# sql-machine-learning/elasticdl

Hardware: NVIDIA B200
Metric: deepfm_train_samples_per_sec (higher is better)
Workload: dtype f32

## Files before the change

elasticdl_b200/_lib.py:

```python
import ctypes
import os

from elasticdl_b200 import build as _build

MAX_SHARDS = 16
MAX_SEGS = 96

OK, EINVAL, ECUDA, ENOTFOUND, EWIDTH, ERANGE, ESTATE = 0, -1, -2, -3, -4, -5, -6


class Seg(ctypes.Structure):
    _fields_ = [
        ("table", ctypes.c_int32),
        ("n", ctypes.c_int32),
        ("ids_dev", ctypes.c_void_p),
        ("n_dev", ctypes.c_void_p),
        ("rows_dev", ctypes.c_void_p),
    ]


class DeepFMArgs(ctypes.Structure):
    _fields_ = [
        ("G", ctypes.c_int32), ("B", ctypes.c_int32),
        ("inv", ctypes.c_void_p), ("n_unique", ctypes.c_void_p),
        ("bet_wide", ctypes.c_void_p), ("bet_deep", ctypes.c_void_p),
        ("dense", ctypes.c_void_p), ("labels", ctypes.c_void_p),
        ("params", ctypes.c_void_p), ("grads", ctypes.c_void_p),
        ("gsum_wide", ctypes.c_void_p), ("gsum_deep", ctypes.c_void_p),
        ("loss", ctypes.c_void_p), ("logits", ctypes.c_void_p), ("scratch", ctypes.c_void_p),
    ]


class PSError(RuntimeError):
    def __init__(self, code, msg):
        super().__init__("b200ps error %d: %s" % (code, msg))
        self.code = code


class PSNotFound(PSError, KeyError):
    pass


class PSRangeError(PSError, ValueError):
    pass


_vp, _i, _i64, _f, _sz = ctypes.c_void_p, ctypes.c_int, ctypes.c_int64, ctypes.c_float, ctypes.c_size_t
_segp = ctypes.POINTER(Seg)
SYMBOLS = {
    "b200ps_last_error": (ctypes.c_char_p, []),
    "b200ps_abi_version": (_i, []),
    "b200ps_create": (_i, [_i, _i, ctypes.c_char_p, ctypes.c_char_p, _i, ctypes.c_uint, ctypes.POINTER(_vp)]),
    "b200ps_destroy": (_i, [_vp]),
    "b200ps_clone_view": (_i, [_vp, _i, ctypes.POINTER(_vp)]),
    "b200ps_shard_create_local": (_i, [_vp, _i, _i]),
    "b200ps_shard_export": (_i, [_vp, _i, _vp, _sz, ctypes.POINTER(_sz)]),
    "b200ps_shard_import": (_i, [_vp, _i, _vp, _sz]),
    "b200ps_table_register": (_i, [_vp, ctypes.c_char_p, _i, ctypes.c_char_p, _i64, ctypes.c_uint64]),
    "b200ps_table_register_pair": (_i, [_vp, ctypes.c_char_p, ctypes.c_char_p, ctypes.c_char_p, _i64, ctypes.c_uint64]),
    "b200ps_table_register_hashed": (_i, [_vp, ctypes.c_char_p, _i, ctypes.c_char_p, _i64, ctypes.c_uint64]),
    "b200ps_dense_register": (_i, [_vp, ctypes.c_char_p, _i, _i64, _i]),
    "b200ps_lookup": (_i, [_vp, ctypes.c_char_p]),
    "b200ps_commit": (_i, [_vp]),
    "b200ps_pull_rows": (_i, [_vp, _segp, _i, _vp]),
    "b200ps_set_rows": (_i, [_vp, _segp, _i, _vp]),
    "b200ps_pull_rows_pair": (_i, [_vp, _segp, ctypes.POINTER(_vp), _i, _vp]),
    "b200ps_push_rows_pair": (_i, [_vp, _segp, ctypes.POINTER(_vp), _i, _vp]),
    "b200ps_xchg_create": (_i, [_vp, _i, _i, ctypes.POINTER(ctypes.c_int32), ctypes.POINTER(ctypes.c_int32)]),
    "b200ps_xchg_pull": (_i, [_vp, _vp, _vp, _vp, _vp, _vp]),
    "b200ps_xchg_profile": (_i, [_vp, _vp, _vp, _vp, _vp, _vp, _vp, ctypes.POINTER(ctypes.c_float), _vp]),
    "b200ps_xchg_push": (_i, [_vp, _vp, _vp, _vp]),
    "b200ps_pull_dense": (_i, [_vp, _segp, _i, _vp]),
    "b200ps_set_dense": (_i, [_vp, _segp, _i, _vp]),
    "b200ps_slot_rows": (_i, [_vp, _i, _i, _segp, _i, _vp]),
    "b200ps_slot_dense": (_i, [_vp, _i, _i, _segp, _i, _vp]),
    "b200ps_push_begin": (_i, [_vp, _f, ctypes.POINTER(ctypes.c_int32), _vp]),
    "b200ps_push_rows": (_i, [_vp, _segp, _i, _vp]),
    "b200ps_push_dense": (_i, [_vp, _segp, _i, _vp]),
    "b200ps_push_dense_reduce": (_i, [_vp, _i, ctypes.POINTER(_vp), _i, _f, _vp]),
    "b200ps_push_end": (_i, [_vp, _vp, _vp]),
    "b200ps_bump_step": (_i, [_vp, _vp]),
    "b200ps_push_begin_shard": (_i, [_vp, _i, _f, ctypes.POINTER(ctypes.c_int32), _vp]),
    "b200ps_push_end_shard": (_i, [_vp, _i, _vp]),
    "b200ps_raw_register": (_i, [_vp, ctypes.c_char_p, _sz]),
    "b200ps_raw_ptr": (_i, [_vp, _i, _i, ctypes.POINTER(_vp), ctypes.POINTER(_sz)]),
    "b200ps_barrier": (_i, [_vp, _vp]),
    "b200ps_kernel_sgd": (_i, [_vp, _vp, _f, ctypes.c_longlong, _vp]),
    "b200ps_kernel_momentum": (_i, [_vp, _vp, _vp, _f, _i, _f, ctypes.c_longlong, _vp]),
    "b200ps_kernel_adam": (_i, [_vp, _vp, _vp, _vp, _f, ctypes.c_longlong, ctypes.c_longlong, _f, _f, _f, _vp, _vp]),
    "b200ps_kernel_adagrad": (_i, [_vp, _vp, _vp, _f, ctypes.c_longlong, _f, _vp]),
    "b200ps_unique_workspace": (_sz, [_i, _i64]),
    "b200ps_unique": (_i, [_vp, _vp, _i, _i64, _vp, _vp, _vp, _vp, _sz, _vp]),
    "b200ps_unique_bounded_workspace": (_sz, [_i, _i64, ctypes.POINTER(_i64)]),
    "b200ps_unique_bounded": (_i, [_vp, _vp, _i, _i64, ctypes.POINTER(_i64), _vp, _vp, _vp, _vp, _sz, _vp]),
    "b200ps_unique_bounded_i32": (_i, [_vp, _vp, _i, _i64, ctypes.POINTER(_i64), _vp, _vp, _vp, _vp, _sz, _vp]),
    "b200ps_unique_bounded_ex": (_i, [_vp, _vp, _i, _i, _i64, ctypes.POINTER(_i64), _vp, _vp, _vp, _vp, _sz, _i, _vp]),
    "b200ps_debug_buffer": (_i, [_vp, _sz]),
    "b200ps_unique_packed": (_i, [_vp, _vp, ctypes.POINTER(ctypes.c_int32), _i, _i64, ctypes.POINTER(_i64), _vp, _vp, _vp, _vp,
                                  _sz, _i, _vp]),
    "b200ps_packed_ids_bytes": (_sz, [ctypes.POINTER(ctypes.c_int32), _i, _i64]),
    "b200ps_segment_sum": (_i, [_vp, _vp, _vp, _i, _i64, _i, _vp, _vp]),
    "b200ps_gather_rows": (_i, [_vp, _vp, _vp, _i, _i64, _i, _vp, _vp]),
    "b200ps_shard_state": (_i, [_vp, _i, ctypes.POINTER(ctypes.c_int32), ctypes.POINTER(_i64), ctypes.POINTER(ctypes.c_int32)]),
    "b200ps_set_shard_state": (_i, [_vp, _i, ctypes.c_int32, _i64, ctypes.c_int32]),
    "b200ps_snapshot_state": (_i, [_vp, _vp, _vp]),
    "b200ps_try_init": (_i, [_vp, _i, ctypes.POINTER(_i)]),
    "b200ps_finish_init": (_i, [_vp, _i, ctypes.c_int32, _vp]),
    "b200ps_table_size": (_i, [_vp, _i, _i, ctypes.POINTER(_i64)]),
    "b200ps_table_ids": (_i, [_vp, _i, _i, _vp, _i64, ctypes.POINTER(_i64)]),
    "b200ps_check": (_i, [_vp]),
    "b200ps_launch_count": (_i64, [_vp]),
    "b200_deepfm_param_count": (_sz, [_i]),
    "b200_deepfm_fwd_bwd": (_i, [ctypes.POINTER(DeepFMArgs), _vp]),
    "b200_deepfm_forward": (_i, [ctypes.POINTER(DeepFMArgs), _vp]),
    "b200_deepfm_fwd_bwd_mma": (_i, [ctypes.POINTER(DeepFMArgs), _vp]),
    "b200_deepfm_mma_launch_count": (_i64, []),
    "b200_deepfm_launch_count": (_i64, []),
    "b200_deepfm_fwd_bwd_tile": (_i, [ctypes.POINTER(DeepFMArgs), _vp]),
    "b200_deepfm_forward_tile": (_i, [ctypes.POINTER(DeepFMArgs), _vp]),
    "b200_deepfm_publish_loss": (_i, [_vp, _vp, _i, _vp, _vp]),
    "b200_deepfm_tile_prologue": (_i, [ctypes.POINTER(DeepFMArgs), _vp]),
    "b200_deepfm_tile_main": (_i, [ctypes.POINTER(DeepFMArgs), _vp]),
    "b200_deepfm_tile_launch_count": (_i64, []),
    "b200_deepfm_tile_last_error": (ctypes.c_char_p, []),
    "b200feat_last_error": (ctypes.c_char_p, []),
    "b200feat_transform": (_i, [_vp, _i, _vp, _i, _vp, _i, _vp, _i, _i, _vp, _i, _i, _i64, _vp, _i, _vp, _vp]),
    "b200feat_hash_strings": (_i, [_vp, _i, _i64, _i64, _vp, _vp]),
    "b200feat_hash_ints": (_i, [_vp, _i64, _i64, _vp, _vp]),
    "b200feat_bucketize": (_i, [_vp, _i64, _vp, _i, _vp, _vp]),
    "b200feat_fingerprint64": (_i, [_vp, _i, _i64, _vp, _vp]),
    "b200feat_launch_count": (_i64, []),
}

_lib = None


def lib():
    global _lib
    if _lib is None:
        path = _build.LIB
        if not os.path.exists(path) or _build._stale():
            path = _build.build()
        handle = ctypes.CDLL(path)
        for name, (res, args) in SYMBOLS.items():
            fn = getattr(handle, name)
            fn.restype = res
            fn.argtypes = args
        if handle.b200ps_abi_version() != 1:
            raise ImportError("libb200ps.so ABI version mismatch")
        _lib = handle
    return _lib


def check(rc):
    if rc >= 0:
        return rc
    msg = lib().b200ps_last_error().decode("utf-8", "replace")
    if rc == ENOTFOUND:
        raise PSNotFound(rc, msg)
    if rc == ERANGE:
        raise PSRangeError(rc, msg)
    if rc in (EINVAL, EWIDTH):
        raise ValueError("b200ps error %d: %s" % (rc, msg))
    raise PSError(rc, msg)
```

elasticdl_b200/csrc/deepfm_tower2.cu:

```cuda
#include <cuda_runtime.h>

#include <cstdlib>
#include <string>

#include "../../include/b200_deepfm.h"

namespace {

constexpr int ND = B200_DEEPFM_NDENSE, D = B200_DEEPFM_DIM, H1 = B200_DEEPFM_H1, H2 = B200_DEEPFM_H2;
constexpr int WD_PAD = 16;
constexpr int TS = 32;
constexpr int THREADS = 256;
constexpr int NKP = 8;
constexpr int KPC = 40;
constexpr int NCOL = 320;
constexpr int XS = 324;
constexpr int RS = 39;
constexpr int RW = H1 + D + 2;
constexpr int MS = 44;
constexpr int MAXG = 38;

struct Layout {
  int in, o_wd, o_w1, o_b1, o_w2, o_b2, o_w3, total;
};
__host__ __device__ inline Layout layout(int G) {
  Layout l;
  l.in = ND + G * D;
  l.o_wd = 0;
  l.o_w1 = WD_PAD;
  l.o_b1 = l.o_w1 + H1 * l.in;
  l.o_w2 = l.o_b1 + H1;
  l.o_b2 = l.o_w2 + H2 * H1;
  l.o_w3 = l.o_b2 + H2;
  l.total = l.o_w3 + H2;
  return l;
}

long long g_launches = 0;
thread_local std::string g_msg;

constexpr int SM_W1X = NCOL * H1;
constexpr int SM_X = TS * XS;
constexpr int SM_P = NKP * RW * TS;
constexpr int SM_R = 2 * TS * RS;
constexpr int SM_WV = MAXG * TS;
constexpr int SM_SMALL = 128;
constexpr size_t SMEM_BYTES = (size_t)(SM_W1X + SM_X + SM_P + SM_R + SM_WV + SM_SMALL) * sizeof(float);

__device__ __forceinline__ void cp_async16(void* smem, const void* gmem) {
  const unsigned s = (unsigned)__cvta_generic_to_shared(smem);
  asm volatile("cp.async.cg.shared.global [%0], [%1], 16;" ::"r"(s), "l"(gmem) : "memory");
}
__device__ __forceinline__ void cp_async4(void* smem, const void* gmem) {
  const unsigned s = (unsigned)__cvta_generic_to_shared(smem);
  asm volatile("cp.async.ca.shared.global [%0], [%1], 4;" ::"r"(s), "l"(gmem) : "memory");
}
__device__ __forceinline__ void cp_async_wait_all() { asm volatile("cp.async.wait_all;" ::: "memory"); }

__host__ __device__ inline int w1x_src(const Layout& l, int G, int c, int j) {
  const int ndeep = G * D;
  if (c < ndeep) return l.o_w1 + j * l.in + ND + c;
  if (c >= MAXG * D && c < MAXG * D + ND) return l.o_w1 + j * l.in + (c - MAXG * D);
  if (c == MAXG * D + ND) return l.o_b1 + j;
  return -1;
}

__global__ void __launch_bounds__(256) k_tile_prep(b200_deepfm_args_t a, int n_params, float* w1x, int main_grid) {
  const long long stride = (long long)gridDim.x * blockDim.x;
  const long long tid = (long long)blockIdx.x * blockDim.x + threadIdx.x;
  if (tid == 0 && a.loss) *a.loss = 0.f;
  if (tid == 0 && blockIdx.y == 0) reinterpret_cast<int*>(w1x + NCOL * H1)[0] = main_grid;
  if (blockIdx.y == 0) {
    if (a.grads)
      for (long long i = tid; i < n_params; i += stride) a.grads[i] = 0.f;
    const Layout l = layout(a.G);
    for (long long i = tid; i < (long long)NCOL * H1; i += stride) {
      const int c = (int)(i / H1), j = (int)(i - (long long)c * H1);
      const int src = w1x_src(l, a.G, c, j);
      w1x[i] = src >= 0 ? a.params[src] : 0.f;
    }
  }
  if (a.gsum_deep == nullptr) return;
  for (int g = blockIdx.y; g < a.G; g += gridDim.y) {
    const int u = a.n_unique[g];
    float* gw = a.gsum_wide + (long long)g * a.B;
    float4* gd = reinterpret_cast<float4*>(a.gsum_deep + (long long)g * a.B * D);
    for (long long i = tid; i < u; i += stride) gw[i] = 0.f;
    for (long long i = tid; i < 2LL * u; i += stride) gd[i] = make_float4(0.f, 0.f, 0.f, 0.f);
  }
}

template <bool BACKWARD>
__global__ void __launch_bounds__(THREADS, 2) k_tower_tile(b200_deepfm_args_t a, const float* __restrict__ w1x_g) {
  extern __shared__ __align__(16) float smem[];
  float* W1x = smem;
  float* X = W1x + SM_W1X;
  float* P = X + SM_X;
  int* Rt0 = reinterpret_cast<int*>(P + SM_P);
  float* WV = reinterpret_cast<float*>(Rt0 + SM_R);
  float* small = WV + SM_WV;
  float* s_w2 = small;
  float* s_b2 = small + 64;
  float* s_w3 = small + 68;
  float* s_wd = small + 72;
  float* T = P;
  float* Mst = P + RW * TS + 64;

  const Layout l = layout(a.G);
  const int B = a.B, G = a.G;
  const int t = threadIdx.x, lane = t & 31, warp = t >> 5;
  {
    const float4* src = reinterpret_cast<const float4*>(w1x_g);
    float4* dst = reinterpret_cast<float4*>(W1x);
    for (int i = t; i < SM_W1X / 4; i += THREADS) dst[i] = src[i];
    for (int i = t; i < H2 * H1; i += THREADS) s_w2[i] = a.params[l.o_w2 + i];
    if (t < H2) { s_b2[t] = a.params[l.o_b2 + t]; s_w3[t] = a.params[l.o_w3 + t]; }
    if (t < ND) s_wd[t] = a.params[l.o_wd + t];
  }
  float2 acc0[H1 / 2], acc1[2];
  float sacc = 0.f;
#pragma unroll
  for (int j = 0; j < H1 / 2; ++j) acc0[j] = make_float2(0.f, 0.f);
  acc1[0] = acc1[1] = make_float2(0.f, 0.f);
  float loss_acc = 0.f;
  __syncthreads();

  const long long ntile = ((long long)B + TS - 1) / TS;
  auto fetch_ranks = [&](const long long tl, int* dst) {
    const long long bb0 = tl * TS;
    for (int i = t; i < G * TS; i += THREADS) {
      long long b = bb0 + (i & 31);
      if (b >= B) b = B - 1;
      cp_async4(dst + (i & 31) * RS + (i >> 5), a.inv + (long long)(i >> 5) * B + b);
    }
  };
  __shared__ int s_tile[2];
  int* tile_counter = reinterpret_cast<int*>(const_cast<float*>(w1x_g) + SM_W1X);
  if (t == 0) {
    s_tile[0] = (int)blockIdx.x;
    s_tile[1] = atomicAdd(tile_counter, 1);
  }
  int cur = 0;
  if ((long long)blockIdx.x < ntile) fetch_ranks(blockIdx.x, Rt0);
  cp_async_wait_all();
  __syncthreads();
  for (int iter = 0;; ++iter, cur ^= 1) {
    const int tile = s_tile[iter & 1], tile_next = s_tile[(iter + 1) & 1];
    if (tile >= ntile) break;
    const long long b0 = (long long)tile * TS;
    int* Rt = Rt0 + cur * (TS * RS);
    {
      const int npair = G * TS;
      constexpr int NFILL = (TS * 16 + THREADS - 1) / THREADS;
      float dv[NFILL];
#pragma unroll
      for (int jj = 0; jj < NFILL; ++jj) {
        const int i = t + THREADS * jj;
        const int s = i >> 4, c = i & 15;
        long long b = b0 + s;
        if (b >= B) b = B - 1;
        float v = c == ND ? 1.0f : 0.f;
        if (i < TS * 16 && c < ND) v = a.dense[b * ND + c];
        dv[jj] = v;
      }
      const int nchunk = G * 2;
      for (int i = t; i < TS * nchunk; i += THREADS) {
        const int s = i / nchunk, ch = i - s * nchunk;
        const int g = ch >> 1;
        const int r = Rt[s * RS + g];
        cp_async16(X + s * XS + ch * 4, a.bet_deep + ((long long)g * B + r) * D + (ch & 1) * 4);
      }
      for (int i = t; i < npair; i += THREADS) {
        const int g = i >> 5, s = i & 31;
        cp_async4(WV + g * TS + s, a.bet_wide + (long long)g * B + Rt[s * RS + g]);
      }
      if (tile_next < ntile) fetch_ranks(tile_next, Rt0 + (cur ^ 1) * (TS * RS));
#pragma unroll
      for (int jj = 0; jj < NFILL; ++jj) {
        const int i = t + THREADS * jj;
        if (i < TS * 16) X[(i >> 4) * XS + MAXG * D + (i & 15)] = dv[jj];
      }
      for (int i = t; i < TS * (MAXG - G) * D; i += THREADS) {
        const int s = i / ((MAXG - G) * D), c = G * D + i % ((MAXG - G) * D);
        X[s * XS + c] = 0.f;
      }
      cp_async_wait_all();
    }
    __syncthreads();
    if (t == 0) s_tile[iter & 1] = atomicAdd(tile_counter, 1);
    const bool live = b0 + lane < B;
    {
      float2 h2[H1 / 2];
#pragma unroll
      for (int j = 0; j < H1 / 2; ++j) h2[j] = make_float2(0.f, 0.f);
      float sd[D], q = 0.f, lin = 0.f;
#pragma unroll
      for (int d = 0; d < D; ++d) sd[d] = 0.f;
      const float* xrow = X + lane * XS;
      const int c0 = warp * KPC;
#pragma unroll
      for (int gi = 0; gi < KPC / D; ++gi) {
        const int c = c0 + gi * D;
        const float4 xa = *reinterpret_cast<const float4*>(xrow + c);
        const float4 xb = *reinterpret_cast<const float4*>(xrow + c + 4);
        const float xv[D] = {xa.x, xa.y, xa.z, xa.w, xb.x, xb.y, xb.z, xb.w};
        const int g = c / D;
        if (g < G) {
#pragma unroll
          for (int d = 0; d < D; ++d) { sd[d] += xv[d]; q = fmaf(xv[d], xv[d], q); }
          lin += WV[g * TS + lane];
        } else if (c == MAXG * D) {
#pragma unroll
          for (int d = 0; d < D; ++d) lin = fmaf(s_wd[d], xv[d], lin);
        } else if (c == MAXG * D + D) {
#pragma unroll
          for (int d = 0; d < ND - D; ++d) lin = fmaf(s_wd[D + d], xv[d], lin);
        }
#pragma unroll
        for (int d = 0; d < D; ++d) {
          const float4* w4 = reinterpret_cast<const float4*>(W1x + (c + d) * H1);
          const float2 xx = make_float2(xv[d], xv[d]);
#pragma unroll
          for (int qd = 0; qd < 4; ++qd) {
            const float4 w = w4[qd];
            h2[2 * qd] = __ffma2_rn(make_float2(w.x, w.y), xx, h2[2 * qd]);
            h2[2 * qd + 1] = __ffma2_rn(make_float2(w.z, w.w), xx, h2[2 * qd + 1]);
          }
        }
      }
      float* mine = P + (warp * RW) * TS + lane;
#pragma unroll
      for (int j = 0; j < H1 / 2; ++j) {
        mine[(2 * j) * TS] = h2[j].x;
        mine[(2 * j + 1) * TS] = h2[j].y;
      }
#pragma unroll
      for (int d = 0; d < D; ++d) mine[(H1 + d) * TS] = sd[d];
      mine[(H1 + D) * TS] = q;
      mine[(H1 + D + 1) * TS] = lin;
    }
    __syncthreads();
    float tsum[4];
#pragma unroll
    for (int i = 0; i < 4; ++i) {
      const int r = warp + 8 * i;
      float v = 0.f;
      if (r < RW) {
#pragma unroll
        for (int kp = 0; kp < NKP; ++kp) v += P[(kp * RW + r) * TS + lane];
      }
      tsum[i] = v;
    }
    __syncthreads();
#pragma unroll
    for (int i = 0; i < 4; ++i) {
      const int r = warp + 8 * i;
      if (r < RW) T[r * TS + lane] = tsum[i];
    }
    __syncthreads();
    float hpre[H1], sd[D];
#pragma unroll
    for (int j = 0; j < H1; ++j) hpre[j] = T[j * TS + lane];
#pragma unroll
    for (int d = 0; d < D; ++d) sd[d] = T[(H1 + d) * TS + lane];
    const float q = T[(H1 + D) * TS + lane], lin = T[(H1 + D + 1) * TS + lane];
    float a1[H1];
#pragma unroll
    for (int j = 0; j < H1; ++j) a1[j] = fmaxf(hpre[j], 0.f);
    float h2[H2], dnn = 0.f;
#pragma unroll
    for (int k = 0; k < H2; ++k) {
      float accv = s_b2[k];
#pragma unroll
      for (int j = 0; j < H1; ++j) accv = fmaf(s_w2[k * H1 + j], a1[j], accv);
      h2[k] = fmaxf(accv, 0.f);
      dnn = fmaf(s_w3[k], h2[k], dnn);
    }
    float ss = 0.f;
#pragma unroll
    for (int d = 0; d < D; ++d) ss = fmaf(sd[d], sd[d], ss);
    const float z = lin + dnn + 0.5f * (ss - q);
    if (warp == 0 && live && a.logits != nullptr) a.logits[b0 + lane] = z;
    float dz = 0.f, dh1[H1];
    if (BACKWARD) {
      const long long bb = live ? b0 + lane : B - 1;
      const float y = a.labels[bb];
      const float lb = fmaxf(z, 0.f) - z * y + log1pf(expf(-fabsf(z)));
      if (warp == 0 && live) loss_acc += lb;
      const float pr = 1.f / (1.f + expf(-z));
      dz = live ? (pr - y) / (float)B : 0.f;
      float dh2[H2];
#pragma unroll
      for (int k = 0; k < H2; ++k) dh2[k] = h2[k] > 0.f ? dz * s_w3[k] : 0.f;
#pragma unroll
      for (int j = 0; j < H1; ++j) {
        float accv = 0.f;
#pragma unroll
        for (int k = 0; k < H2; ++k) accv = fmaf(s_w2[k * H1 + j], dh2[k], accv);
        dh1[j] = hpre[j] > 0.f ? accv : 0.f;
      }
      if (warp == 0) {
        float4* m4 = reinterpret_cast<float4*>(Mst + lane * MS);
#pragma unroll
        for (int qd = 0; qd < 4; ++qd) m4[qd] = make_float4(dh1[4 * qd], dh1[4 * qd + 1], dh1[4 * qd + 2], dh1[4 * qd + 3]);
#pragma unroll
        for (int qd = 0; qd < 4; ++qd) m4[4 + qd] = make_float4(a1[4 * qd], a1[4 * qd + 1], a1[4 * qd + 2], a1[4 * qd + 3]);
        m4[8] = make_float4(dh2[0], dh2[1], dh2[2], dh2[3]);
        m4[9] = make_float4(h2[0], h2[1], h2[2], h2[3]);
        m4[10] = make_float4(dz, 0.f, 0.f, 0.f);
      }
      const float* xrow = X + lane * XS;
#pragma unroll 1
      for (int gi = 0; gi < KPC / D; ++gi) {
        const int g = warp * (KPC / D) + gi;
        if (g >= G) break;
        const int c = g * D;
        const float4 xa = *reinterpret_cast<const float4*>(xrow + c);
        const float4 xb = *reinterpret_cast<const float4*>(xrow + c + 4);
        const float ev[D] = {xa.x, xa.y, xa.z, xa.w, xb.x, xb.y, xb.z, xb.w};
        float x[D + 1];
#pragma unroll
        for (int d = 0; d < D; ++d) {
          const float4* w4 = reinterpret_cast<const float4*>(W1x + (c + d) * H1);
          float2 dt2 = make_float2(0.f, 0.f);
#pragma unroll
          for (int qd = 0; qd < 4; ++qd) {
            const float4 w = w4[qd];
            dt2 = __ffma2_rn(make_float2(w.x, w.y), make_float2(dh1[4 * qd + 0], dh1[4 * qd + 1]), dt2);
            dt2 = __ffma2_rn(make_float2(w.z, w.w), make_float2(dh1[4 * qd + 2], dh1[4 * qd + 3]), dt2);
          }
          x[d] = fmaf(dz, sd[d] - ev[d], dt2.x + dt2.y);
        }
        x[D] = dz;
        const int r = Rt[lane * RS + g];
        const int key = live ? r : -1 - lane;
        const unsigned peers = __match_any_sync(0xffffffffu, key);
        const int rank = __popc(peers & ((1u << lane) - 1));
        const int maxn = __reduce_max_sync(0xffffffffu, (unsigned)__popc(peers));
        const unsigned above = peers & ~((2u << lane) - 1);
        int nxt = above ? __ffs(above) - 1 : -1;
        for (int step = 1; step < maxn; step <<= 1) {
          const int src = nxt >= 0 ? nxt : lane;
          const bool take = nxt >= 0 && (rank & (2 * step - 1)) == 0;
#pragma unroll
          for (int e = 0; e <= D; ++e) {
            const float yv = __shfl_sync(0xffffffffu, x[e], src);
            if (take) x[e] += yv;
          }
          const int nn = __shfl_sync(0xffffffffu, nxt, src);
          nxt = nxt >= 0 ? nn : -1;
        }
        if (live && rank == 0) {
          float* od = a.gsum_deep + ((long long)g * B + r) * D;
          atomicAdd(reinterpret_cast<float4*>(od), make_float4(x[0], x[1], x[2], x[3]));
          atomicAdd(reinterpret_cast<float4*>(od + 4), make_float4(x[4], x[5], x[6], x[7]));
          atomicAdd(a.gsum_wide + (long long)g * B + r, x[D]);
        }
      }
      __syncthreads();
      {
        const int c1 = 256 + (t & 63), jsel = t >> 6;
#pragma unroll 4
        for (int s = 0; s < TS; ++s) {
          const float4* d4 = reinterpret_cast<const float4*>(Mst + s * MS);
          const float4 q0 = d4[0], q1 = d4[1], q2 = d4[2], q3 = d4[3];
          const float dh[H1] = {q0.x, q0.y, q0.z, q0.w, q1.x, q1.y, q1.z, q1.w, q2.x, q2.y, q2.z, q2.w, q3.x, q3.y, q3.z, q3.w};
          const float x0 = X[s * XS + t], x1 = X[s * XS + c1];
          const float4 dq = jsel == 0 ? q0 : (jsel == 1 ? q1 : (jsel == 2 ? q2 : q3));
          const float2 xx0 = make_float2(x0, x0), xx1 = make_float2(x1, x1);
#pragma unroll
          for (int j = 0; j < H1 / 2; ++j) acc0[j] = __ffma2_rn(make_float2(dh[2 * j], dh[2 * j + 1]), xx0, acc0[j]);
          acc1[0] = __ffma2_rn(make_float2(dq.x, dq.y), xx1, acc1[0]);
          acc1[1] = __ffma2_rn(make_float2(dq.z, dq.w), xx1, acc1[1]);
        }
        if (t < H2 * H1 + 2 * H2 + ND) {
          const int o = t;
          for (int s = 0; s < TS; ++s) {
            const float* m = Mst + s * MS;
            float v;
            if (o < H2 * H1) v = m[32 + o / H1] * m[16 + o % H1];
            else if (o < H2 * H1 + H2) v = m[32 + o - H2 * H1];
            else if (o < H2 * H1 + 2 * H2) v = m[40] * m[36 + o - H2 * H1 - H2];
            else v = m[40] * X[s * XS + MAXG * D + o - H2 * H1 - 2 * H2];
            sacc += v;
          }
        }
      }
    }
    __syncthreads();
  }
  if (BACKWARD) {
#pragma unroll
    for (int j = 0; j < H1; ++j) {
      const int dst = w1x_src(l, G, t, j);
      if (dst >= 0) atomicAdd(a.grads + dst, (j & 1) ? acc0[j >> 1].y : acc0[j >> 1].x);
    }
#pragma unroll
    for (int j = 0; j < 4; ++j) {
      const int dst = w1x_src(l, G, 256 + (t & 63), (t >> 6) * 4 + j);
      if (dst >= 0) atomicAdd(a.grads + dst, (j & 1) ? acc1[j >> 1].y : acc1[j >> 1].x);
    }
    if (t < H2 * H1 + 2 * H2 + ND) {
      const int o = t;
      int off;
      if (o < H2 * H1) off = l.o_w2 + o;
      else if (o < H2 * H1 + H2) off = l.o_b2 + o - H2 * H1;
      else if (o < H2 * H1 + 2 * H2) off = l.o_w3 + o - H2 * H1 - H2;
      else off = l.o_wd + o - H2 * H1 - 2 * H2;
      atomicAdd(a.grads + off, sacc);
    }
    if (warp == 0) {
      for (int o = 16; o > 0; o >>= 1) loss_acc += __shfl_down_sync(0xffffffffu, loss_acc, o);
      if (lane == 0) atomicAdd(a.loss, loss_acc / (float)B);
    }
  }
}

__global__ void k_publish_loss(const float* __restrict__ loss, float* ring, int ring_len, unsigned* cursor) {
  const unsigned at = *cursor;
  *reinterpret_cast<volatile float*>(ring + (at % (unsigned)ring_len)) = *loss;
  *cursor = at + 1;
}

int check_args(const b200_deepfm_args_t* a, bool backward) {
  if (!a || a->G < 1 || a->B < 1) { g_msg = "bad shape"; return -1; }
  if (a->G > MAXG) { g_msg = "the tile tower holds at most 38 id groups"; return -1; }
  if (!a->inv || !a->bet_wide || !a->bet_deep || !a->dense || !a->params || !a->scratch) { g_msg = "null input"; return -1; }
  if (backward && (!a->labels || !a->grads || !a->gsum_wide || !a->gsum_deep || !a->loss || !a->n_unique)) {
    g_msg = "null output";
    return -1;
  }
  return 0;
}

template <bool BACKWARD>
int launch(const b200_deepfm_args_t* args, void* stream, int what = 3) {
  cudaStream_t st = (cudaStream_t)stream;
  int dev = 0, n_sm = 148;
  cudaGetDevice(&dev);
  cudaDeviceGetAttribute(&n_sm, cudaDevAttrMultiProcessorCount, dev);
  static bool attr_done[64][2] = {};
  if (dev < 64 && !attr_done[dev][BACKWARD]) {
    cudaFuncSetAttribute(k_tower_tile<BACKWARD>, cudaFuncAttributeMaxDynamicSharedMemorySize, (int)SMEM_BYTES);
    attr_done[dev][BACKWARD] = true;
  }
  b200_deepfm_args_t a = *args;
  if (!BACKWARD) { a.grads = nullptr; a.gsum_deep = nullptr; a.gsum_wide = nullptr; a.loss = nullptr; }
  float* w1x = a.scratch;
  const long long ntile = ((long long)a.B + TS - 1) / TS;
  static const int per_sm = [] { const char* e = getenv("B200_TILE_CTAS"); const int v = e ? atoi(e) : 2; return v < 1 ? 1 : v; }();
  long long grid = (long long)n_sm * per_sm;
  if (grid > ntile) grid = ntile;
  if (what & 1) {
    k_tile_prep<<<dim3(4, BACKWARD ? a.G : 1), 256, 0, st>>>(a, layout(a.G).total, w1x, (int)grid);
    g_launches += 1;
  }
  if (!(what & 2)) {
    cudaError_t e = cudaGetLastError();
    if (e != cudaSuccess) { g_msg = cudaGetErrorString(e); return -2; }
    return 0;
  }
  k_tower_tile<BACKWARD><<<(unsigned)grid, THREADS, SMEM_BYTES, st>>>(*args, w1x);
  g_launches += 1;
  cudaError_t e = cudaGetLastError();
  if (e != cudaSuccess) { g_msg = cudaGetErrorString(e); return -2; }
  return 0;
}

}

extern "C" {

int64_t b200_deepfm_tile_launch_count(void) { return g_launches; }
const char* b200_deepfm_tile_last_error(void) { return g_msg.c_str(); }

int b200_deepfm_fwd_bwd_tile(const b200_deepfm_args_t* args, void* stream) {
  if (check_args(args, true)) return -1;
  return launch<true>(args, stream);
}

int b200_deepfm_tile_prologue(const b200_deepfm_args_t* args, void* stream) {
  if (check_args(args, true)) return -1;
  return launch<true>(args, stream, 1);
}

int b200_deepfm_tile_main(const b200_deepfm_args_t* args, void* stream) {
  if (check_args(args, true)) return -1;
  return launch<true>(args, stream, 2);
}

int b200_deepfm_publish_loss(const float* loss_dev, float* ring_host_mapped, int ring_len, unsigned* cursor_dev, void* stream) {
  if (!loss_dev || !ring_host_mapped || ring_len < 1 || !cursor_dev) { g_msg = "bad publish_loss arguments"; return -1; }
  k_publish_loss<<<1, 1, 0, (cudaStream_t)stream>>>(loss_dev, ring_host_mapped, ring_len, cursor_dev);
  g_launches += 1;
  cudaError_t e = cudaGetLastError();
  if (e != cudaSuccess) { g_msg = cudaGetErrorString(e); return -2; }
  return 0;
}

int b200_deepfm_forward_tile(const b200_deepfm_args_t* args, void* stream) {
  if (check_args(args, false) || !args->logits) return -1;
  return launch<false>(args, stream);
}

}
```

include/b200_deepfm.h:

```cpp
#ifndef B200_DEEPFM_H_
#define B200_DEEPFM_H_
#include <stddef.h>
#include <stdint.h>
#ifdef __cplusplus
extern "C" {
#endif

#define B200_DEEPFM_NDENSE 13
#define B200_DEEPFM_DIM 8
#define B200_DEEPFM_H1 16
#define B200_DEEPFM_H2 4
#define B200_DEEPFM_SCRATCH 44

typedef struct {
  int32_t G;
  int32_t B;
  const int32_t* inv;
  const int32_t* n_unique;
  const float* bet_wide;
  const float* bet_deep;
  const float* dense;
  const float* labels;
  const float* params;
  float* grads;
  float* gsum_wide;
  float* gsum_deep;
  float* loss;
  float* logits;
  float* scratch;
} b200_deepfm_args_t;

size_t b200_deepfm_param_count(int G);
int b200_deepfm_fwd_bwd(const b200_deepfm_args_t* args, void* stream);
int b200_deepfm_fwd_bwd_mma(const b200_deepfm_args_t* args, void* stream);
int64_t b200_deepfm_mma_launch_count(void);
int b200_deepfm_fwd_bwd_tile(const b200_deepfm_args_t* args, void* stream);
int b200_deepfm_forward_tile(const b200_deepfm_args_t* args, void* stream);
int b200_deepfm_publish_loss(const float* loss_dev, float* ring_host_mapped, int ring_len, unsigned* cursor_dev, void* stream);
int b200_deepfm_tile_prologue(const b200_deepfm_args_t* args, void* stream);
int b200_deepfm_tile_main(const b200_deepfm_args_t* args, void* stream);
int64_t b200_deepfm_tile_launch_count(void);
const char* b200_deepfm_tile_last_error(void);
int b200_deepfm_forward(const b200_deepfm_args_t* args, void* stream);
int64_t b200_deepfm_launch_count(void);

#ifdef __cplusplus
}
#endif
#endif
```

Measured before the change: 204.3 million.

## Accumulate per-row gradients in shared memory for small-vocab fields; add phase timestamps

Adds a per-CTA shared-memory accumulator for row gradients of fields whose unique count fits in the tile, so each row update is a shared atomic instead of a warp-match plus global atomic. The accumulator is flushed to global gsum once per CTA at the end, skipping zero entries. It also adds optional globaltimer phase stamps written to a new stamps field in the args struct. The extra shared memory may reduce occupancy, and shared atomic contention on hot rows could cost time.

```diff
diff --git a/elasticdl_b200/_lib.py b/elasticdl_b200/_lib.py
--- a/elasticdl_b200/_lib.py
+++ b/elasticdl_b200/_lib.py
@@ -28,6 +28,7 @@
         ("params", ctypes.c_void_p), ("grads", ctypes.c_void_p),
         ("gsum_wide", ctypes.c_void_p), ("gsum_deep", ctypes.c_void_p),
         ("loss", ctypes.c_void_p), ("logits", ctypes.c_void_p), ("scratch", ctypes.c_void_p),
+        ("stamps", ctypes.c_void_p),
     ]
 
 
diff --git a/elasticdl_b200/csrc/deepfm_tower2.cu b/elasticdl_b200/csrc/deepfm_tower2.cu
--- a/elasticdl_b200/csrc/deepfm_tower2.cu
+++ b/elasticdl_b200/csrc/deepfm_tower2.cu
@@ -45,7 +45,10 @@
 constexpr int SM_R = 2 * TS * RS;
 constexpr int SM_WV = MAXG * TS;
 constexpr int SM_SMALL = 128;
-constexpr size_t SMEM_BYTES = (size_t)(SM_W1X + SM_X + SM_P + SM_R + SM_WV + SM_SMALL) * sizeof(float);
+constexpr int SACC_ROWS = 256, SACC_W = D + 1;
+constexpr int SM_ACC = SACC_ROWS * SACC_W;
+constexpr size_t SMEM_BYTES = (size_t)(SM_W1X + SM_X + SM_P + SM_R + SM_WV + SM_SMALL + SM_ACC) * sizeof(float);
+static_assert(SMEM_BYTES + 1024 <= 113 * 1024, "two CTAs per SM");
 
 __device__ __forceinline__ void cp_async16(void* smem, const void* gmem) {
   const unsigned s = (unsigned)__cvta_generic_to_shared(smem);
@@ -56,6 +59,12 @@
   asm volatile("cp.async.ca.shared.global [%0], [%1], 4;" ::"r"(s), "l"(gmem) : "memory");
 }
 __device__ __forceinline__ void cp_async_wait_all() { asm volatile("cp.async.wait_all;" ::: "memory"); }
+__device__ __forceinline__ long long global_ns() {
+  long long v;
+  asm volatile("mov.u64 %0, %%globaltimer;" : "=l"(v));
+  return v;
+}
+enum { PH_GATHER = 0, PH_FORWARD, PH_MIDDLE, PH_ROWGRAD, PH_PARAMGRAD, PH_TILES, PH_SLOTS = 8 };
 
 __host__ __device__ inline int w1x_src(const Layout& l, int G, int c, int j) {
   const int ndeep = G * D;
@@ -103,6 +112,7 @@
   float* s_b2 = small + 64;
   float* s_w3 = small + 68;
   float* s_wd = small + 72;
+  float* s_acc = small + SM_SMALL;
   float* T = P;
   float* Mst = P + RW * TS + 64;
 
@@ -123,6 +133,19 @@
   for (int j = 0; j < H1 / 2; ++j) acc0[j] = make_float2(0.f, 0.f);
   acc1[0] = acc1[1] = make_float2(0.f, 0.f);
   float loss_acc = 0.f;
+  __shared__ int s_off[MAXG];
+  if (BACKWARD) {
+    for (int i = t; i < SM_ACC; i += THREADS) s_acc[i] = 0.f;
+    if (t == 0) {
+      int off = 0;
+      for (int g = 0; g < G; ++g) {
+        const int u = a.n_unique[g];
+        const bool fits = u <= TS && off + u <= SACC_ROWS;
+        s_off[g] = fits ? off : -1;
+        if (fits) off += u;
+      }
+    }
+  }
   __syncthreads();
 
   const long long ntile = ((long long)B + TS - 1) / TS;
@@ -135,6 +158,15 @@
     }
   };
   __shared__ int s_tile[2];
+  __shared__ long long s_ph[PH_SLOTS], s_ph_t;
+  auto stamp = [&](int slot) {
+    if (a.stamps != nullptr && t == 0) {
+      const long long now = global_ns();
+      s_ph[slot] += now - s_ph_t;
+      s_ph_t = now;
+    }
+  };
+  if (a.stamps != nullptr && t < PH_SLOTS) s_ph[t] = 0;
   int* tile_counter = reinterpret_cast<int*>(const_cast<float*>(w1x_g) + SM_W1X);
   if (t == 0) {
     s_tile[0] = (int)blockIdx.x;
@@ -149,6 +181,7 @@
     if (tile >= ntile) break;
     const long long b0 = (long long)tile * TS;
     int* Rt = Rt0 + cur * (TS * RS);
+    if (a.stamps != nullptr && t == 0) { s_ph_t = global_ns(); s_ph[PH_TILES] += 1; }
     {
       const int npair = G * TS;
       constexpr int NFILL = (TS * 16 + THREADS - 1) / THREADS;
@@ -187,6 +220,7 @@
       cp_async_wait_all();
     }
     __syncthreads();
+    stamp(PH_GATHER);
     if (t == 0) s_tile[iter & 1] = atomicAdd(tile_counter, 1);
     const bool live = b0 + lane < B;
     {
@@ -240,6 +274,7 @@
       mine[(H1 + D + 1) * TS] = lin;
     }
     __syncthreads();
+    stamp(PH_FORWARD);
     float tsum[4];
 #pragma unroll
     for (int i = 0; i < 4; ++i) {
@@ -309,6 +344,7 @@
         m4[9] = make_float4(h2[0], h2[1], h2[2], h2[3]);
         m4[10] = make_float4(dz, 0.f, 0.f, 0.f);
       }
+      stamp(PH_MIDDLE);
       const float* xrow = X + lane * XS;
 #pragma unroll 1
       for (int gi = 0; gi < KPC / D; ++gi) {
@@ -333,6 +369,15 @@
         }
         x[D] = dz;
         const int r = Rt[lane * RS + g];
+        const int so = s_off[g];
+        if (so >= 0) {
+          if (live) {
+            float* acc = s_acc + (so + r) * SACC_W;
+#pragma unroll
+            for (int e = 0; e <= D; ++e) atomicAdd(acc + e, x[e]);
+          }
+          continue;
+        }
         const int key = live ? r : -1 - lane;
         const unsigned peers = __match_any_sync(0xffffffffu, key);
         const int rank = __popc(peers & ((1u << lane) - 1));
@@ -358,6 +403,7 @@
         }
       }
       __syncthreads();
+      stamp(PH_ROWGRAD);
       {
         const int c1 = 256 + (t & 63), jsel = t >> 6;
 #pragma unroll 4
@@ -388,8 +434,25 @@
       }
     }
     __syncthreads();
+    stamp(BACKWARD ? PH_PARAMGRAD : PH_MIDDLE);
+  }
+  if (a.stamps != nullptr) {
+    __syncthreads();
+    if (t < PH_SLOTS) a.stamps[(long long)blockIdx.x * PH_SLOTS + t] = s_ph[t];
   }
   if (BACKWARD) {
+    for (int g = 0; g < G; ++g) {
+      const int so = s_off[g];
+      if (so < 0) continue;
+      const int n = a.n_unique[g] * SACC_W;
+      for (int i = t; i < n; i += THREADS) {
+        const float v = s_acc[so * SACC_W + i];
+        if (v == 0.f) continue;
+        const int r = i / SACC_W, e = i - r * SACC_W;
+        if (e < D) atomicAdd(a.gsum_deep + ((long long)g * B + r) * D + e, v);
+        else atomicAdd(a.gsum_wide + (long long)g * B + r, v);
+      }
+    }
 #pragma unroll
     for (int j = 0; j < H1; ++j) {
       const int dst = w1x_src(l, G, t, j);
diff --git a/include/b200_deepfm.h b/include/b200_deepfm.h
--- a/include/b200_deepfm.h
+++ b/include/b200_deepfm.h
@@ -28,6 +28,7 @@
   float* loss;
   float* logits;
   float* scratch;
+  int64_t* stamps;
 } b200_deepfm_args_t;
 
 size_t b200_deepfm_param_count(int G);
```

Measured after the change: 145.5 million (median of 6 runs). 28.8% lower.
